# ZhenlongYuan/DVP-MVS

Hardware: AMD Instinct MI355X
Metric: Mpixels/sec/PatchMatch-iteration (higher is better)
Workload: dtype f32

## Files before the change

### __graft_entry__.py

```python
import importlib
import os
import subprocess
import sys

ROOT = os.path.dirname(os.path.abspath(__file__))
if ROOT not in sys.path:
    sys.path.insert(0, ROOT)


def build() -> None:
    subprocess.check_call(["make", "-s", "-C", os.path.join(ROOT, "dvp-mvs_amd", "csrc")])
    host = os.path.join(ROOT, "dvp-mvs_amd", "host")
    if os.path.exists(os.path.join(host, "Makefile")):
        subprocess.check_call(["make", "-s", "-C", host])
    subprocess.check_call(["make", "-s", "-C", os.path.join(ROOT, "oracle")])
    subprocess.check_call(["make", "-s", "-C", os.path.join(ROOT, "tests", "emul")])
    subprocess.check_call(["make", "-s", "-C", os.path.join(ROOT, "tests", "host")])
    subprocess.check_call(["make", "-s", "-C", os.path.join(ROOT, "tests", "half16")])
    subprocess.check_call(["make", "-s", "-C", os.path.join(ROOT, "tests", "jpeg_host")])
    subprocess.check_call(["make", "-s", "-C", os.path.join(ROOT, "tests", "edges_host")])
    subprocess.check_call(["make", "-s", "-C", os.path.join(ROOT, "tests", "viewclean_host")])
    subprocess.check_call(["make", "-s", "-C", os.path.join(ROOT, "tests", "labels_host")])
    subprocess.check_call(["make", "-s", "-C", os.path.join(ROOT, "tests", "pyramid_host")])
    subprocess.check_call(["make", "-s", "-C", os.path.join(ROOT, "tests", "prior_host")])
    subprocess.check_call(["make", "-s", "-C", os.path.join(ROOT, "tests", "reuse_host")])
    subprocess.check_call(["make", "-s", "-C", os.path.join(ROOT, "tests", "devmem_host")])
    subprocess.check_call(["make", "-s", "-C", os.path.join(ROOT, "tests", "jpeg_dec_host")])
    subprocess.check_call(["make", "-s", "-C", os.path.join(ROOT, "tests", "convert_host")])
    subprocess.check_call(["make", "-s", "-C", os.path.join(ROOT, "tests", "undistort_host")])
    pkg = importlib.import_module("dvp-mvs_amd")
    lib = pkg.get_capi().lib()
    missing = [s for s in pkg.get_capi().EXPORTS + pkg.get_capi().EXPORTS_WITH_DIGITS if not hasattr(lib, s)]
    if missing:
        raise RuntimeError("libdvp_mvs_hip.so lacks symbols: %s" % missing)


def smoke() -> None:
    import numpy as np
    pkg = importlib.import_module("dvp-mvs_amd")
    synth, capi = pkg.synth, pkg.get_capi()
    from oracle import oracle as O
    W, H, S = 96, 64, 3
    sc = synth.make_scene(W, H, S)
    p = synth.default_params(S + 1, max_iterations=1, state=synth.FIRST_INIT, use_APD=0)
    p["depth_min"] = np.float32(2.5) * np.float32(0.6)
    p["depth_max"] = np.float32(6.5) * np.float32(1.2)
    state = dict(planes=np.zeros((H * W, 4), np.float32), edge=sc["edge"], label=sc["label"],
                 radius=np.full(H * W, 5, np.int32))
    g = capi.from_scene(sc, p, device=0)
    g.upload_state(**state)
    g.run_patchmatch()
    o = O.from_scene(sc, p)
    o.upload_state(**state)
    o.run_patchmatch()
    pg, po = g.get("planes"), o.get("planes")
    same = (pg.view(np.uint32) == po.view(np.uint32)) | (np.isnan(pg) & np.isnan(po))
    if not same.all():
        raise AssertionError("smoke: HIP planes differ from the oracle in %d values" % int((~same).sum()))
    for n in ("selected_views", "weak_info", "radius"):
        if not (g.get(n) == o.get(n)).all():
            raise AssertionError("smoke: %s differs from the oracle" % n)
    print("smoke ok: %dx%d S=%d bit-exact vs oracle; total %.2f ms" % (W, H, S, g.timings()["total_ms"]))


if __name__ == "__main__":
    build()
    if os.path.exists("/dev/kfd"):
        smoke()
```

### dvp-mvs_amd/csrc/dvp_engine.hip

```cpp
#include "dvp_stages.hpp"
#include "dvp_jpeg_enc.h"
#include "dvp_edges_run.h"
#include "dvp_viewclean_run.h"
#include "dvp_prior_run.h"
#include "dvp_pyramid_run.h"
#include <hip/hip_runtime.h>
#include <cstdlib>
#include <string>
#include <vector>
#include <cstdio>
#include <cstring>
#include <mutex>
#include <condition_variable>
#include <thread>
#include <chrono>
#include <algorithm>
#include <cmath>

using namespace dvp;

struct LaunchArgs {
	int tiles_x, tiles, rows, half, colour, iter;
};

// ... 520 lines not shown
}

extern "C" __global__ void __launch_bounds__(256) dvp_gen_candidates_views(const Dev d, const LaunchArgs a) {
	int px, py;
	if (block_to_pixel(blockIdx.x, threadIdx.x & 63, threadIdx.x >> 6, a.tiles_x, a.tiles, a.rows, 0, 0, d.width, d.height, &px, &py))
		gen_candidates_views_px<kCandGroup>(d, px, py, (int)blockIdx.y * kCandGroup);
}
extern "C" __global__ void __launch_bounds__(256) dvp_gen_candidates_views_list(const Dev d, const unsigned* list, const unsigned* n_list) {
	const unsigned t = blockIdx.x * 256 + threadIdx.x;
	if (t >= *n_list) return;
	const int center = (int)list[t];
	const int py = center / d.width, px = center - py * d.width;
	gen_candidates_views_px<kCandGroup>(d, px, py, (int)blockIdx.y * kCandGroup);
}

extern "C" __global__ void __launch_bounds__(256) dvp_anchor_mask(const Dev d, const ListArgs a, uint8_t* mask) {
	const int t = blockIdx.x * 256 + threadIdx.x;
	if (t >= a.count) return;
	const int center = d.weak_list[a.base + t];
	const s2* nb = d.neighbours + (size_t)d.neighbours_map[center] * DVP_NEIGHBOUR_NUM;
	for (int k = 1; k < DVP_NEIGHBOUR_NUM; ++k) {
		const s2 q = nb[k];
		if (q.x >= 0 && q.y >= 0 && q.x < d.width && q.y < d.height) mask[(size_t)q.y * d.width + q.x] = 1;
	}
}
extern "C" __global__ void __launch_bounds__(256) dvp_mask_compact(const uint8_t* mask, size_t L, unsigned* list, unsigned* n_list) {
	const size_t p = (size_t)blockIdx.x * 256 + threadIdx.x;
	const bool go = p < L && mask[p] != 0;
	const unsigned long long m = __ballot(go);
	if (!m) return;
	const int lane = threadIdx.x & 63;
	unsigned base = 0;
	if (lane == __builtin_ctzll(m)) base = atomicAdd(n_list, (unsigned)__popcll(m));
	base = __shfl(base, __builtin_ctzll(m), 64);
	if (go) list[base + __popcll(m & ((1ull << lane) - 1ull))] = (unsigned)p;
}
extern "C" __global__ void __launch_bounds__(256) dvp_gen_candidates_list(const Dev d, const unsigned* list, const unsigned* n_list) {
	const unsigned t = blockIdx.x * 256 + threadIdx.x;
	if (t >= *n_list) return;
	const int center = (int)list[t];
	const int py = center / d.width, px = center - py * d.width;
	gen_candidates_px(d, px, py, (int)blockIdx.y);
}

extern "C" __global__ void dvp_pack_bits_transposed(const uint8_t* __restrict__ map, uint32_t* __restrict__ bits, int W, int H, int tiles_x, size_t words, int equals) {
	const size_t w = (size_t)blockIdx.x * blockDim.x + threadIdx.x;
	if (w < words) bits[w] = pack_edge_word_t(map, W, H, tiles_x, w, equals);
}

extern "C" __global__ void dvp_edge_cell_counts(const Dev d) {
	const int c = blockIdx.x * blockDim.x + threadIdx.x;
	if (c >= d.sat_cells_x * d.sat_cells_y) return;
	const int cy = c / d.sat_cells_x, cx = c - cy * d.sat_cells_x;
	int n = 0;
	for (int r = 0; r < 8; ++r) {
		const int y = cy * 8 + r;
		if (y >= d.height) break;
		const unsigned w = d.edge_bits[(size_t)(((y >> 5) * d.edge_tiles_x + (cx >> 2)) * 32 + (y & 31))];
		n += __popc((w >> ((cx & 3) * 8)) & 255u);
	}
	d.edge_sat[(cy + 1) * (d.sat_cells_x + 1) + cx + 1] = n;
}
extern "C" __global__ void dvp_edge_sat_rows(const Dev d) {
	const int r = blockIdx.x * blockDim.x + threadIdx.x;
	if (r > d.sat_cells_y) return;
	int* row = d.edge_sat + (size_t)r * (d.sat_cells_x + 1);
	int acc = 0;
	for (int x = 0; x <= d.sat_cells_x; ++x) { acc += (r == 0 || x == 0) ? 0 : row[x]; row[x] = acc; }
}
extern "C" __global__ void dvp_edge_sat_cols(const Dev d) {
	const int x = blockIdx.x * blockDim.x + threadIdx.x;
	if (x > d.sat_cells_x) return;
	const int P = d.sat_cells_x + 1;
	int acc = 0;
	for (int r = 0; r <= d.sat_cells_y; ++r) { acc += d.edge_sat[(size_t)r * P + x]; d.edge_sat[(size_t)r * P + x] = acc; }
}

extern "C" __global__ void __launch_bounds__(256) dvp_strong_search(const Dev d, const LaunchArgs a) {
	int px, py;
	if (block_to_pixel(blockIdx.x, threadIdx.x & 63, threadIdx.x >> 6, a.tiles_x, a.tiles, a.rows, a.half, a.colour, d.width, d.height, &px, &py))
		strong_search_px(d, px, py);
}

extern "C" __global__ void __launch_bounds__(256) dvp_strong_plan(const Dev d, const LaunchArgs a) {
	int px, py;
	if (block_to_pixel(blockIdx.x, threadIdx.x & 63, threadIdx.x >> 6, a.tiles_x, a.tiles, a.rows, a.half, a.colour, d.width, d.height, &px, &py) &&
	    d.weak_info[px + py * d.width] != DVP_WEAK)
		strong_plan_px(d, px, py);
}

extern "C" __global__ void __launch_bounds__(256) dvp_edge_rays(const Dev d, int what) {
	edge_ray_line(d, blockIdx.y, blockIdx.x * blockDim.x + threadIdx.x, what);
}

constexpr int kWeakTile = 16, kWeakSuper = 64, kWeakChunk = 1024;
DVP_HD void weak_slot_origin(int slot, int supers_x, int* tx, int* ty) {
	const int super = slot >> 4, t = slot & 15;
	*tx = (super % supers_x) * kWeakSuper + (t & 3) * kWeakTile;
	*ty = (super / supers_x) * kWeakSuper + (t >> 2) * kWeakTile;
}
extern "C" __global__ void __launch_bounds__(256) dvp_weak_counts(const uint8_t* __restrict__ weak, int W, int H, int supers_x, int n_slots, int n_chunks, int* __restrict__ counts) {
	const int lane = threadIdx.x & 63;
	const int unit = blockIdx.x * 4 + (threadIdx.x >> 6);
	if (unit < n_slots) {
		int tx, ty;
		weak_slot_origin(unit, supers_x, &tx, &ty);
		int nb = 0, nr = 0;
		for (int step = 0; step < 4; ++step) {
			const int x = tx + (lane & 15), y = ty + step * 4 + (lane >> 4);
			const bool wk = x < W && y < H && weak[(size_t)y * W + x] == DVP_WEAK;
			nb += __popcll(__ballot(wk && !((x + y) & 1)));
			nr += __popcll(__ballot(wk && ((x + y) & 1)));
		}
		if (lane == 0) { counts[unit] = nb; counts[n_slots + unit] = nr; }
	} else if (unit < n_slots + n_chunks) {
		const int chunk = unit - n_slots;
		const size_t L = (size_t)W * H;
		int n = 0;
		for (int step = 0; step < kWeakChunk / 64; ++step) {
			const size_t i = (size_t)chunk * kWeakChunk + step * 64 + lane;
			n += __popcll(__ballot(i < L && weak[i] == DVP_WEAK));
		}
		if (lane == 0) counts[2 * n_slots + chunk] = n;
	}
}
extern "C" __global__ void __launch_bounds__(1024) dvp_scan3(int* __restrict__ data, int s0, int s1, int s2, int s3, int* __restrict__ totals) {
	__shared__ int part[1024];
	__shared__ int carry;
	const int starts[4] = { s0, s1, s2, s3 };
	const int lo = starts[blockIdx.x], hi = starts[blockIdx.x + 1];
	if (threadIdx.x == 0) carry = 0;
	__syncthreads();
	for (int base = lo; base < hi; base += 1024) {
		const int i = base + (int)threadIdx.x;
		const int v = i < hi ? data[i] : 0;
		part[threadIdx.x] = v;
		__syncthreads();
		for (int off = 1; off < 1024; off <<= 1) {
			const int add = threadIdx.x >= (unsigned)off ? part[threadIdx.x - off] : 0;
			__syncthreads();
			part[threadIdx.x] += add;
			__syncthreads();
		}
		if (i < hi) data[i] = carry + part[threadIdx.x] - v;
		__syncthreads();
		if (threadIdx.x == 1023) carry += part[1023];
		__syncthreads();
	}
	if (threadIdx.x == 0) totals[blockIdx.x] = carry;
}
extern "C" __global__ void __launch_bounds__(256) dvp_weak_fill(const uint8_t* __restrict__ weak, int W, int H, int supers_x, int n_slots, int n_chunks,
                                                               const int* __restrict__ offs, const int* __restrict__ totals, int* __restrict__ list, int* __restrict__ map) {
	const int lane = threadIdx.x & 63;
	const int unit = blockIdx.x * 4 + (threadIdx.x >> 6);
	const unsigned long long below = (1ull << lane) - 1ull;
	if (unit < n_slots) {
		int tx, ty;
		weak_slot_origin(unit, supers_x, &tx, &ty);
		int ob = offs[unit], orr = totals[0] + offs[n_slots + unit];
		for (int step = 0; step < 4; ++step) {
			const int x = tx + (lane & 15), y = ty + step * 4 + (lane >> 4);
			const bool wk = x < W && y < H && weak[(size_t)y * W + x] == DVP_WEAK;
			const bool red = (x + y) & 1;
			const unsigned long long mb = __ballot(wk && !red), mr = __ballot(wk && red);
			if (wk) list[red ? orr + __popcll(mr & below) : ob + __popcll(mb & below)] = y * W + x;
			ob += __popcll(mb);
			orr += __popcll(mr);
// ... 908 lines not shown
		make_sector_taps(p->weak_radius, &taps, &start);
		if (dalloc(c, &c->sector_taps, taps.size(), false) || dalloc(c, &c->sector_start, start.size(), false)) return 1;
		HIP_TRY(c, hipMemcpyAsync(c->sector_taps, taps.data(), taps.size() * 4, hipMemcpyHostToDevice, c->stream));
		HIP_TRY(c, hipMemcpyAsync(c->sector_start, start.data(), start.size() * 4, hipMemcpyHostToDevice, c->stream));
		HIP_TRY(c, hipStreamSynchronize(c->stream));
		c->lut_radius = p->weak_radius;
	}
	sync_dev_struct(c);
	return 0;
}
int dvp_set_seed(dvp_ctx* c, uint64_t seed) { c->d.seed = seed; return 0; }
int dvp_set_sampler(dvp_ctx* c, int s) { c->d.sampler = s ? 1 : 0; bump_reuse_epoch(c); return 0; }
int dvp_set_profiling(dvp_ctx* c, int on) { c->profiling = on != 0; sync_dev_struct(c); return 0; }


static size_t alloc_group_or_fall_back(dvp_ctx* c, std::initializer_list<AllocReq> reqs, const char* hook, bool* fits, const char* msg, double gb, size_t retry_bytes = 0) {
	void* got[4] = { nullptr, nullptr, nullptr, nullptr };
	const AllocReq* r = reqs.begin();
	const size_t n = reqs.size();
	size_t first = r[0].bytes;
	bool ok = n <= 4 && !(hook && getenv(hook));
	for (size_t i = 0; i < n && ok; ++i) {
		if (!r[i].p) continue;
		ok = hipMalloc(&got[i], r[i].bytes) == hipSuccess;
		if (!ok && i == 0 && retry_bytes) { (void)hipGetLastError(); first = retry_bytes; ok = hipMalloc(&got[0], first) == hipSuccess; }
		if (!ok) got[i] = nullptr;
		else if (r[i].zero) ok = hipMemsetAsync(got[i], 0, r[i].bytes, c->stream) == hipSuccess;
	}
	if (!ok) {
		(void)hipGetLastError();
		for (void* q : got) if (q) (void)hipFree(q);
		*fits = false;
		if (msg) fprintf(stderr, msg, gb);
	}
	else for (size_t i = 0; i < n; ++i) if (r[i].p) { *r[i].p = got[i]; c->allocs.push_back(got[i]); }
	sync_dev_struct(c);
	return ok ? first : 0;
}

static int grow_anchor_table(dvp_ctx* c, size_t wc) {
	const size_t need = wc * (size_t)(c->NI - 1) * kAnchors;
	if (anchor_table_off(c) || need <= c->anchor_tab_alloc) return 0;
	HIP_TRY(c, hipStreamSynchronize(c->stream));
	dfree(c, &c->anchor_tab);
	c->anchor_tab_alloc = 0;
	c->anchor_tab_alloc = alloc_group_or_fall_back(c, { areq(&c->anchor_tab, (need + need / 2) * sizeof(AnchorRec)) }, nullptr, &c->anchor_tab_fits,
		"dvp: no room for the weak update's anchor table (%.1f GB); forming the reference side per item\n", (double)need * sizeof(AnchorRec) / 1e9,
		need * sizeof(AnchorRec)) / sizeof(AnchorRec);
	return 0;
}
static int ensure_anchor_table(dvp_ctx* c, int covered_rows) {
	if (anchor_table_off(c) || c->anchor_tab_valid) return 0;
	const int wc = c->d.weak_black + c->d.weak_red;
	if (grow_anchor_table(c, (size_t)wc)) return 1;
	if (anchor_table_off(c)) return 0;
	c->anchor_tab_valid = true;
	sync_dev_struct(c);
	ListArgs la;
	la.base = 0; la.count = wc; la.iter = 0; la.covered_rows = covered_rows;
	const long long n = (long long)wc * (c->NI - 1) * kAnchors;
	if (n > 0) {
		hipLaunchKernelGGL(dvp_weak_anchor_table, dim3((unsigned)((n + 255) / 256)), dim3(256), 0, c->stream, c->d, la);
		HIP_TRY(c, hipGetLastError());
	}
	return 0;
}

static int grow_weak_phase_buffers(dvp_ctx* c, size_t wc) {
	if (!c->sw.weak_phased || !c->weak_phase_fits || wc <= c->weak_phase_alloc) return 0;
	HIP_TRY(c, hipStreamSynchronize(c->stream));
	dfree(c, &c->weak_rec); dfree(c, &c->weak_ctab); dfree(c, &c->weak_ev);
	c->weak_phase_alloc = 0;
	const size_t cap = std::min<size_t>(c->L, wc + wc / 2), S = (size_t)c->NI - 1;
	if (alloc_group_or_fall_back(c, { areq(&c->weak_rec, cap * sizeof(WeakRec)), areq(&c->weak_ctab, cap * kTaps * kTaps * sizeof(f2)), areq(&c->weak_ev, cap * 8 * S * sizeof(float)) },
			"DVP_TEST_WEAK_PHASE_ALLOC_FAIL", &c->weak_phase_fits, "dvp: no room for the phased weak update's hand-over buffers (%.2f GB); using the one-wave kernel\n", (double)cap * (sizeof(WeakRec) + 288 + 32 * S) / 1e9))
		c->weak_phase_alloc = cap;
	return 0;
}

static void ensure_strong_reuse_buffers(dvp_ctx* c) {
	if (c->reuse_costs || !c->sw.strong_reuse || !c->reuse_fits || strong_form(c->sw, c->NI - 1, c->split_fits, false, 0).kernel != STRONG_SPLIT) return;
	const size_t L = c->L, vec = (size_t)kSlotCount * (c->NI - 1) * L * sizeof(float) + 64 ;
	const size_t Lh = (size_t)((c->W + 1) / 2) * c->H;
	alloc_group_or_fall_back(c, { areq(&c->reuse_costs, vec), areq(&c->reuse_keys, L * kSlotCount * sizeof(PlaneKey)), areq(&c->reuse_hdr, L * sizeof(ReuseHdr), true),
			c->strong_rec ? AllocReq{} : areq(&c->strong_rec, (size_t)SR_FIELDS * Lh * sizeof(*c->strong_rec)) },
		"DVP_TEST_REUSE_ALLOC_FAIL", &c->reuse_fits, "dvp: no room for the strong update's plane cache (%.1f GB); every visit evaluates all its planes\n", (double)(vec + L * (kSlotCount * sizeof(PlaneKey) + sizeof(ReuseHdr))) / 1e9);
}
static void ensure_strong_split_buffers(dvp_ctx* c) {
	if (c->slot_costs || strong_form(c->sw, c->NI - 1, c->split_fits, false, 0).kernel != STRONG_SPLIT) return;
	if (!getenv("DVP_TEST_SPLIT_ALLOC_FAIL")) {
		ensure_strong_reuse_buffers(c);
		if (c->reuse_costs) return;
	}
	const size_t Lh = (size_t)((c->W + 1) / 2) * c->H;
	alloc_group_or_fall_back(c, { areq(&c->slot_costs, (size_t)kSlotCount * (c->NI - 1) * Lh * sizeof(*c->slot_costs) + 64 ),
			areq(&c->strong_rec, (size_t)SR_FIELDS * Lh * sizeof(*c->strong_rec)) },
		"DVP_TEST_SPLIT_ALLOC_FAIL", &c->split_fits, "dvp: no room for the split strong update's cost buffer (%.1f GB); using the monolithic kernel\n", (double)kSlotCount * (c->NI - 1) * Lh * 4 / 1e9);
}
static void ensure_sweep_buffers(dvp_ctx* c) {
	if (c->sweep_cost || !c->sw.sweep_split || !c->sweep_fits) return;
	const size_t L = c->L;
	c->sweep_band_rows = sweep_band_rows(c->sw, c->W, c->H, c->NI - 1);
	const size_t band_px = c->sweep_band_rows > 0 ? (size_t)c->sweep_band_rows * c->W : L;
	alloc_group_or_fall_back(c, { areq(&c->sweep_rec, 2 * L * sizeof(f4)), areq(&c->sweep_pc, 61 * L * sizeof(float)), areq(&c->sweep_cost, sweep_cost_floats(band_px, c->NI - 1) * sizeof(float)) },
		"DVP_TEST_SWEEP_ALLOC_FAIL", &c->sweep_fits, "dvp: no room for the view-compacted DepthToWeak's cost buffer (%.1f GB); using the fused kernel\n", (double)(c->NI - 1) * kSweepFields * L * 4 / 1e9);
}


#define DVP_PICK(NAME, SUF) (c->d.sampler ? NAME##_exact##SUF : NAME##SUF)
#define DVP_PICK_FMT(NAME, TAIL) (fmt == 1 ? DVP_PICK(NAME, _u8##TAIL) : (fmt == 2 ? DVP_PICK(NAME, _f16##TAIL) : DVP_PICK(NAME, TAIL)))

static LaunchArgs make_args(const LaunchGeom& g, int colour, int iter) {
	LaunchArgs a;
	a.tiles_x = g.tiles_x; a.tiles = g.tiles; a.rows = g.rows; a.half = g.half ? 1 : 0;
	a.colour = colour; a.iter = iter;
	return a;
}

static void launch_gen_candidates(dvp_ctx* c, hipStream_t stream, const Dev& d, unsigned blocks, const LaunchArgs& a, const unsigned* list = nullptr, const unsigned* n_list = nullptr) {
	const bool all = gen_candidates_all_views(d);
	const dim3 grid(blocks, all ? (unsigned)((c->NI - 1 + kCandGroup - 1) / kCandGroup) : (unsigned)(c->NI - 1)), block(256);
	if (list) hipLaunchKernelGGL(all ? dvp_gen_candidates_views_list : dvp_gen_candidates_list, grid, block, 0, stream, d, list, n_list);
	else hipLaunchKernelGGL(all ? dvp_gen_candidates_views : dvp_gen_candidates, grid, block, 0, stream, d, a);
}

static int launch_strong_prep(dvp_ctx* c, const LaunchGeom& g, const LaunchArgs& a) {
	EventPair prep;
	prep.stage = DVP_ST_STRONG_PREP;
	HIP_TRY(c, hipEventCreate(&prep.a));
	HIP_TRY(c, hipEventCreate(&prep.b));
	HIP_TRY(c, hipEventRecord(prep.a, c->stream));
	HIP_TRY(c, hipMemcpyAsync(c->planes_snap, c->planes, c->L * 16, hipMemcpyDeviceToDevice, c->stream));
	HIP_TRY(c, hipMemcpyAsync(c->costs_snap, c->costs, c->L * 4, hipMemcpyDeviceToDevice, c->stream));
	ensure_strong_split_buffers(c);
	hipLaunchKernelGGL(dvp_strong_search, dim3(g.grid()), dim3(256), 0, c->stream, c->d, a);
	if (strong_form(c->sw, c->NI - 1, c->split_fits, c->d.reuse_hdr != nullptr, 0).plan) hipLaunchKernelGGL(dvp_strong_plan, dim3(g.grid()), dim3(256), 0, c->stream, c->d, a);
	HIP_TRY(c, hipGetLastError());
	HIP_TRY(c, hipEventRecord(prep.b, c->stream));
	c->events.push_back(prep);
	return 0;
}

static int launch_strong_update(dvp_ctx* c, const LaunchGeom& g, const LaunchArgs& a) {
	const dim3 grid(g.grid()), block(256);
	const dim3 wave_grid((unsigned)((g.grid() + 7) / 8 * 32)), wave_block(64);
	ensure_strong_split_buffers(c);
	const StrongForm f = strong_form(c->sw, c->NI - 1, c->split_fits, c->d.reuse_hdr != nullptr, (unsigned long long)c->pitch * (c->H + 2 * kImgPad) * 8 * c->NI);
	switch (f.kernel) {
	case STRONG_SPLIT:
		if (f.eval_items) hipLaunchKernelGGL(DVP_PICK(dvp_strong_eval_items, ), wave_grid, wave_block, 0, c->stream, c->d, a);
		else hipLaunchKernelGGL(DVP_PICK(dvp_strong_eval, ), wave_grid, wave_block, 0, c->stream, c->d, a);
		hipLaunchKernelGGL(f.decide == 4 ? dvp_strong_decide_v4 : f.decide == 6 ? dvp_strong_decide_v6 : f.decide == 8 ? dvp_strong_decide_v8 : f.decide == 10 ? dvp_strong_decide_v10 :
		                   f.decide == 12 ? dvp_strong_decide_v12 : f.decide == 16 ? dvp_strong_decide_v16 : dvp_strong_decide_wide, grid, block, 0, c->stream, c->d, a);
		if (f.refine_lanes) hipLaunchKernelGGL(DVP_PICK(dvp_strong_refine_lanes, ), wave_grid, wave_block, 0, c->stream, c->d, a);
		else hipLaunchKernelGGL(DVP_PICK(dvp_strong_refine, ), wave_grid, wave_block, 0, c->stream, c->d, a);
		break;
	case STRONG_MONO_V8: hipLaunchKernelGGL(DVP_PICK(dvp_strong_update_v8, ), grid, block, 0, c->stream, c->d, a); break;
	case STRONG_MONO_V16: hipLaunchKernelGGL(DVP_PICK(dvp_strong_update_v16, ), grid, block, 0, c->stream, c->d, a); break;
	case STRONG_MONO: hipLaunchKernelGGL(DVP_PICK(dvp_strong_update, ), grid, block, 0, c->stream, c->d, a); break;
	}
	HIP_TRY(c, hipGetLastError());
	return 0;
}

static int launch_weak_update(dvp_ctx* c, ListArgs la) {
	if (ensure_anchor_table(c, la.covered_rows)) return 1;
	if (c->d.anchor_tab && grow_weak_phase_buffers(c, (size_t)(c->d.weak_black + c->d.weak_red))) return 1;
// ... 687 lines not shown
```

### dvp-mvs_amd/csrc/dvp_strong.hpp

```cpp
#ifndef DVP_STRONG_HPP_
#define DVP_STRONG_HPP_

#include "dvp_ncc.hpp"

namespace dvp {

DVP_HD void sort_small(float* v, int n) {
	for (int i = 1; i < n; i++) {
		const float tmp = v[i];
		int j = i;
		for (; j >= 1 && tmp < v[j - 1]; j--) v[j] = v[j - 1];
		v[j] = tmp;
	}
}

DVP_HD f4 random_normal_yzl_sel(const Dev& d, int px, int py, Rng& rng, float depth, uint32_t sel) {
	const int W = d.width, H = d.height;
	const DvpCamera rc = load_camera(d, 0);
	f3 vd[20];
	{
		const f4 v0 = view_direction(rc, px, py, depth);
		vd[0] = mk3(v0.x, v0.y, v0.z);
	}
	int index = 1;
// ... 438 lines not shown
			}
			Rng rd(d.seed, (uint32_t)center, rng_site(PH_STRONG, iter, SUB_DEPTH_RAND));
			Rng rn(d.seed, (uint32_t)center, rng_site(PH_STRONG, iter, SUB_NORMAL));
			Rng rp(d.seed, (uint32_t)center, rng_site(PH_STRONG, iter, SUB_DEPTH_PERT));
			const float depth_rand = rd.uniform() * (P.depth_max - P.depth_min) + P.depth_min;
			if (selected_views_written) d.selected_views[center] = sel_mask;
			const f4 n_rand = random_normal_yzl(d, px, py, rn, depth_now);
			const float dmin_p = (1 - 0.02f) * depth_now, dmax_p = (1 + 0.02f) * depth_now;
			const float depth_pert = rp.uniform() * (dmax_p - dmin_p) + dmin_p;
			f4 n_pert = plane_now;
			normalize3(&n_pert);
			ref_depths[0] = depth_rand; ref_normals[0] = plane_now;
			ref_depths[1] = depth_now;  ref_normals[1] = n_rand;
			ref_depths[2] = depth_rand; ref_normals[2] = n_rand;
			ref_depths[3] = depth_now;  ref_normals[3] = n_pert;
			ref_depths[4] = depth_now;  ref_normals[4] = n_pert;
			ref_depths[5] = depth_pert; ref_normals[5] = plane_now;
		} else {
			float tc = 0.0f;
			for (int j = 0; j < S; ++j)
				if (vw[j] > 0) tc += vw[j] * cv[j];
			tc /= weight_norm;
			const float db = depth_from_plane(rc, plane, px, py);
			if (db >= P.depth_min && db <= P.depth_max && tc < cost_now) {
				depth_now = db;
				plane_now = plane;
				cost_now = tc;
			}
		}
	}

	if (P.state == DVP_REFINE_INIT) {
		if (cost_now < costs_center - 0.1) {
			costs_center = cost_now;
			d.planes[center] = plane_now;
		}
	} else {
		costs_center = cost_now;
		d.planes[center] = plane_now;
	}
	d.costs[center] = costs_center;
}

constexpr int kSlotCur = 16;
constexpr int kSlotCount = 17;
enum { SR_PLANE = 0, SR_DEPTH = 4, SR_COST = 5, SR_CENTER = 6, SR_DRAND = 7, SR_DPERT = 8, SR_NRAND = 9, SR_DUP = 12 , SR_FIELDS = 15 };
DVP_HD size_t half_index(const Dev& d, int px, int py) { return (size_t)py * d.half_w + (size_t)(px >> 1); }
#ifndef DVP_SLOT_LAYOUT
#define DVP_SLOT_LAYOUT 1
#endif
DVP_HD int slot_place(int slot) {
#if DVP_SLOT_LAYOUT
	return slot < 8 ? 2 * slot : (slot < 16 ? 2 * (slot - 8) + 1 : slot);
#else
	return slot;
#endif
}
DVP_HD size_t slot_cost_index(const Dev& d, int slot, int v, int px, int py) {
	const size_t Lh = (size_t)d.half_w * (size_t)d.height;
	const int S = d.params.num_images - 1;
#if DVP_SLOT_LAYOUT
	return (half_index(d, px, py) * kSlotCount + (size_t)slot_place(slot)) * (size_t)S + (size_t)v;
#else
	return (size_t)(slot * S + v) * Lh + half_index(d, px, py);
#endif
}
struct SlotCostView { const float* base; size_t slot_stride, view_stride; };
DVP_HD SlotCostView slot_cost_view(const Dev& d, int px, int py) {
	const size_t Lh = (size_t)d.half_w * (size_t)d.height;
	const int S = d.params.num_images - 1;
	SlotCostView r;
#if DVP_SLOT_LAYOUT
	r.base = d.slot_costs + half_index(d, px, py) * kSlotCount * (size_t)S;
	r.slot_stride = (size_t)S;
	r.view_stride = 1;
#else
	r.base = d.slot_costs + half_index(d, px, py);
	r.slot_stride = (size_t)S * Lh;
	r.view_stride = Lh;
#endif
	return r;
}
DVP_HD bool same_plane_bits(const f4 a, const f4 b) {
	return f32_bits(a.x) == f32_bits(b.x) && f32_bits(a.y) == f32_bits(b.y) && f32_bits(a.z) == f32_bits(b.z) && f32_bits(a.w) == f32_bits(b.w);
}
DVP_HD uint32_t strong_slot_planes(const Dev& d, int center, f4 pl[kSlotCount]) {
	const size_t L = (size_t)d.width * d.height;
	uint32_t have = 0;
#pragma unroll
	for (int slot = 0; slot < kSlotCount; ++slot) {
		const int pos = slot < 16 ? d.search_pos[(size_t)slot * L + center] : center;
		pl[slot] = mk4(0.0f, 0.0f, 0.0f, 0.0f);
		if (pos >= 0) { pl[slot] = d.planes_snap[pos]; have |= 1u << slot; }
	}
	return have;
}
DVP_HD uint32_t strong_slot_sources_of(const f4 pl[kSlotCount], uint32_t have, uint32_t w[3]) {
	uint32_t uniq = 0;
	w[0] = w[1] = w[2] = 0;
#pragma unroll
	for (int slot = 0; slot < kSlotCount; ++slot) {
		int src = slot;
#pragma unroll
		for (int u = slot - 1; u >= 0; --u)
			if (((have >> u) & 1u) && same_plane_bits(pl[u], pl[slot])) src = u;
		if (!((have >> slot) & 1u)) continue;
		if (src == slot) uniq |= 1u << slot;
		if (slot < 8) w[0] |= (uint32_t)src << (4 * slot);
		else if (slot < 16) w[1] |= (uint32_t)src << (4 * (slot - 8));
		else w[2] = (uint32_t)src;
	}
	return uniq;
}
DVP_HD uint32_t strong_slot_sources(const Dev& d, int center, uint32_t w[3]) {
	f4 pl[kSlotCount];
	const uint32_t have = strong_slot_planes(d, center, pl);
	return strong_slot_sources_of(pl, have, w);
}
DVP_HD int strong_slot_source(uint32_t w0, uint32_t w1, uint32_t w2, int slot) {
	return slot < 8 ? (int)((w0 >> (4 * slot)) & 15u) : slot < 16 ? (int)((w1 >> (4 * (slot - 8))) & 15u) : (int)w2;
}
constexpr uint32_t kPlaceMask = (1u << kSlotCount) - 1u;
DVP_HD int strong_slot_place_of(uint32_t w0, uint32_t w1, uint32_t w2, int slot) {
	return slot < 6 ? (int)((w0 >> (5 * slot)) & 31u) : slot < 12 ? (int)((w1 >> (5 * (slot - 6))) & 31u) : (int)((w2 >> (5 * (slot - 12))) & 31u);
}
DVP_HD void strong_source_places(const uint32_t src[3], uint32_t place_w[3]) {
	place_w[0] = place_w[1] = place_w[2] = 0;
#pragma unroll
	for (int s = 0; s < kSlotCount; ++s)
		place_w[s / 6] |= (uint32_t)slot_place(strong_slot_source(src[0], src[1], src[2], s)) << (5 * (s % 6));
}
DVP_HD PlaneKey plane_key(const f4 p) {
	PlaneKey k;
	k.w[0] = f32_bits(p.x); k.w[1] = f32_bits(p.y); k.w[2] = f32_bits(p.z); k.w[3] = f32_bits(p.w);
	return k;
}
DVP_HD uint32_t strong_reuse_plan(const f4 pl[kSlotCount], uint32_t uniq, const uint32_t src[3], PlaneKey* keys, ReuseHdr* hdr,
                                  uint32_t epoch, int radius, uint32_t place_w[3]) {
	const ReuseHdr h = *hdr;
	const uint32_t valid = (h.epoch == epoch && h.radius == (uint32_t)radius) ? (h.valid & kPlaceMask) : 0u;
	int place[kSlotCount];
#pragma unroll
	for (int s = 0; s < kSlotCount; ++s) place[s] = -1;
	uint32_t held = 0;
	if (valid) {
#pragma unroll
		for (int p = 0; p < kSlotCount; ++p) {
			if (!((valid >> p) & 1u)) continue;
			const PlaneKey k = keys[p];
#pragma unroll
			for (int s = 0; s < kSlotCount; ++s) {
				if (!((uniq >> s) & 1u) || place[s] >= 0) continue;
				if (k.w[0] == f32_bits(pl[s].x) && k.w[1] == f32_bits(pl[s].y) && k.w[2] == f32_bits(pl[s].z) && k.w[3] == f32_bits(pl[s].w)) { place[s] = p; held |= 1u << p; }
			}
		}
	}
	uint32_t free_places = kPlaceMask & ~held, eval = 0;
#pragma unroll
	for (int s = 0; s < kSlotCount; ++s) {
		if (!((uniq >> s) & 1u) || place[s] >= 0) continue;
		const int p = dvp_ctz(free_places);
		free_places &= free_places - 1;
		place[s] = p;
		eval |= 1u << s;
		keys[p] = plane_key(pl[s]);
	}
	place_w[0] = place_w[1] = place_w[2] = 0;
#pragma unroll
	for (int s = 0; s < kSlotCount; ++s) {
		const int from = strong_slot_source(src[0], src[1], src[2], s);
		int p = 0;
#pragma unroll
		for (int u = 0; u <= s; ++u)
			if (u == from && place[u] >= 0) p = place[u];
		place_w[s / 6] |= (uint32_t)p << (5 * (s % 6));
	}
	ReuseHdr o;
	o.valid = kPlaceMask & ~free_places; o.radius = (uint32_t)radius; o.epoch = epoch; o.eval = eval;
	*hdr = o;
	return eval;
}
DVP_HD void strong_plan_px(const Dev& d, int px, int py) {
	const int center = py * d.width + px;
	f4 pl[kSlotCount];
	const uint32_t have = strong_slot_planes(d, center, pl);
	uint32_t src[3], pw[3];
	const uint32_t uniq = strong_slot_sources_of(pl, have, src);
	strong_reuse_plan(pl, uniq, src, d.reuse_keys + (size_t)center * kSlotCount, d.reuse_hdr + center, d.reuse_epoch, d.radius[center], pw);
	const size_t Lh = (size_t)d.half_w * (size_t)d.height;
	uint32_t* dup = reinterpret_cast<uint32_t*>(d.strong_rec) + half_index(d, px, py);
	dup[SR_DUP * Lh] = pw[0]; dup[(SR_DUP + 1) * Lh] = pw[1]; dup[(SR_DUP + 2) * Lh] = pw[2];
}
template <int SMP>
DVP_HD void strong_eval_item(const Dev& d, const PatchCtx& c, int px, int py, int slot, bool store, unsigned long long* nevals) {
	const int W = d.width;
	const int center = py * W + px;
	const int S = d.params.num_images - 1;
	const size_t L = (size_t)W * d.height;
	const int pos = slot < 16 ? d.search_pos[(size_t)slot * L + center] : center;
	const f4 plane = d.planes_snap[pos];
	const bool reuse = d.reuse_costs != nullptr;
	float* const buf = reuse ? d.reuse_costs : d.slot_costs;
	int at = slot_place(slot);
	if (reuse) {
		const size_t Lh = (size_t)d.half_w * (size_t)d.height;
		const int word = (slot >= 6) + (slot >= 12);
		const uint32_t pw = reinterpret_cast<const uint32_t*>(d.strong_rec)[(size_t)(SR_DUP + word) * Lh + half_index(d, px, py)];
		at = (int)((pw >> (5 * (slot - 6 * word))) & 31u);
	}
	for (int v = 0; v < S; ++v) {
		const float cost = ncc_old<SMP>(d, c, px, py, v + 1, plane);
#if DVP_SLOT_LAYOUT
		const size_t rec = reuse ? (size_t)center : half_index(d, px, py);
		if (store) DVP_NT_STORE(4, &buf[(rec * kSlotCount + (size_t)at) * (size_t)S + (size_t)v], cost);
#else
		if (store) DVP_NT_STORE(4, &buf[reuse ? ((size_t)center * kSlotCount + (size_t)at) * (size_t)S + (size_t)v : slot_cost_index(d, slot, v, px, py)], cost);
#endif
	}
	if (nevals && store) *nevals += (unsigned long long)S;
}
template <int SMP>
DVP_HD void strong_eval_px(const Dev& d, int px, int py, PatchTab tab, unsigned long long* nevals) {
	const int W = d.width;
	const int center = py * W + px;
	PatchCtx c;
	{
		int radius, inc;
		patch_geometry(d, center, &radius, &inc);
		build_patch_ctx(d, px, py, radius, inc, 0, tab, &c);
	}
	uint32_t uniq;
	if (d.reuse_hdr) uniq = d.reuse_hdr[center].eval;
	else {
		uint32_t src[3], w[3];
		uniq = strong_slot_sources(d, center, src);
		strong_source_places(src, w);
		const size_t Lh = (size_t)d.half_w * (size_t)d.height, hi = half_index(d, px, py);
		uint32_t* dup = reinterpret_cast<uint32_t*>(d.strong_rec) + hi;
		dup[SR_DUP * Lh] = w[0]; dup[(SR_DUP + 1) * Lh] = w[1]; dup[(SR_DUP + 2) * Lh] = w[2];
	}
	for (uint32_t m = uniq; m; m &= m - 1) strong_eval_item<SMP>(d, c, px, py, dvp_ctz(m), true, nevals);
}

template <int MV>
DVP_HD void load_slot_costs(const float* sc, size_t view_stride, int S, float* out) {
#if defined(__HIP_DEVICE_COMPILE__) && DVP_SLOT_LAYOUT
	typedef float f4v __attribute__((ext_vector_type(4), aligned(4)));
	constexpr int Q = (MV + 3) / 4;
	f4v q[Q];
#pragma unroll
	for (int i = 0; i < Q; ++i) q[i] = DVP_NT_LOAD(8, &reinterpret_cast<const f4v*>(sc)[i]);
#pragma unroll
	for (int v = 0; v < MV; ++v) out[v] = v < S ? q[v >> 2][v & 3] : 0.0f;
#else
#pragma unroll
	for (int v = 0; v < MV; ++v) out[v] = v < S ? sc[(size_t)v * view_stride] : 0.0f;
#endif
}

DVP_HD void strong_decide_wide_px(const Dev& d, int px, int py, int iter);
template <int MV>
DVP_HD void strong_decide_px(const Dev& d, int px, int py, int iter) {
#if !defined(__HIP_DEVICE_COMPILE__)
	if (d.params.num_images - 1 > MV) { strong_decide_wide_px(d, px, py, iter); return; }
#endif
	const int W = d.width;
	const int center = py * W + px;
	const DvpParams& P = d.params;
	const DvpCamera rc = load_camera(d, 0);
	const int S = P.num_images - 1;
	const bool reuse = d.reuse_costs != nullptr;
	SlotCostView cv;
// ... 1128 lines not shown
```

Before: 60.91.

## Match strong-plan reuse slots by fingerprint with coalesced key layout

The strong plan kernel now hashes each cached plane key and each candidate plane into a 30-bit fingerprint and matches slots by comparing fingerprints. It falls back to the full bitwise key scan only when a fingerprint match fails verification. The reuse keys move from a per-pixel array of records to a slot-major, colour-split layout, so neighbouring threads read adjacent keys. The change also makes the plane gather branchless, loads the search positions up front, and sets a minimum-occupancy launch bound on the plan kernel. The cost is extra hashing arithmetic and possible register pressure, aimed at cutting the divergent nested compare loops and the strided key loads.

```diff
diff --git a/__graft_entry__.py b/__graft_entry__.py
--- a/__graft_entry__.py
+++ b/__graft_entry__.py
@@ -24,6 +24,7 @@
     subprocess.check_call(["make", "-s", "-C", os.path.join(ROOT, "tests", "pyramid_host")])
     subprocess.check_call(["make", "-s", "-C", os.path.join(ROOT, "tests", "prior_host")])
     subprocess.check_call(["make", "-s", "-C", os.path.join(ROOT, "tests", "reuse_host")])
+    subprocess.check_call(["make", "-s", "-C", os.path.join(ROOT, "tests", "plan_fp_host")])
     subprocess.check_call(["make", "-s", "-C", os.path.join(ROOT, "tests", "devmem_host")])
     subprocess.check_call(["make", "-s", "-C", os.path.join(ROOT, "tests", "jpeg_dec_host")])
     subprocess.check_call(["make", "-s", "-C", os.path.join(ROOT, "tests", "convert_host")])
diff --git a/dvp-mvs_amd/csrc/dvp_engine.hip b/dvp-mvs_amd/csrc/dvp_engine.hip
--- a/dvp-mvs_amd/csrc/dvp_engine.hip
+++ b/dvp-mvs_amd/csrc/dvp_engine.hip
@@ -626,7 +626,10 @@
 		strong_search_px(d, px, py);
 }
 
-extern "C" __global__ void __launch_bounds__(256) dvp_strong_plan(const Dev d, const LaunchArgs a) {
+#ifndef DVP_LB_PLAN
+#define DVP_LB_PLAN 3
+#endif
+extern "C" __global__ void __launch_bounds__(256, DVP_LB_PLAN) dvp_strong_plan(const Dev d, const LaunchArgs a) {
 	int px, py;
 	if (block_to_pixel(blockIdx.x, threadIdx.x & 63, threadIdx.x >> 6, a.tiles_x, a.tiles, a.rows, a.half, a.colour, d.width, d.height, &px, &py) &&
 	    d.weak_info[px + py * d.width] != DVP_WEAK)
@@ -1701,7 +1704,7 @@
 	if (c->reuse_costs || !c->sw.strong_reuse || !c->reuse_fits || strong_form(c->sw, c->NI - 1, c->split_fits, false, 0).kernel != STRONG_SPLIT) return;
 	const size_t L = c->L, vec = (size_t)kSlotCount * (c->NI - 1) * L * sizeof(float) + 64 ;
 	const size_t Lh = (size_t)((c->W + 1) / 2) * c->H;
-	alloc_group_or_fall_back(c, { areq(&c->reuse_costs, vec), areq(&c->reuse_keys, L * kSlotCount * sizeof(PlaneKey)), areq(&c->reuse_hdr, L * sizeof(ReuseHdr), true),
+	alloc_group_or_fall_back(c, { areq(&c->reuse_costs, vec), areq(&c->reuse_keys, 2 * Lh * kSlotCount * sizeof(PlaneKey) ), areq(&c->reuse_hdr, L * sizeof(ReuseHdr), true),
 			c->strong_rec ? AllocReq{} : areq(&c->strong_rec, (size_t)SR_FIELDS * Lh * sizeof(*c->strong_rec)) },
 		"DVP_TEST_REUSE_ALLOC_FAIL", &c->reuse_fits, "dvp: no room for the strong update's plane cache (%.1f GB); every visit evaluates all its planes\n", (double)(vec + L * (kSlotCount * sizeof(PlaneKey) + sizeof(ReuseHdr))) / 1e9);
 }
diff --git a/dvp-mvs_amd/csrc/dvp_strong.hpp b/dvp-mvs_amd/csrc/dvp_strong.hpp
--- a/dvp-mvs_amd/csrc/dvp_strong.hpp
+++ b/dvp-mvs_amd/csrc/dvp_strong.hpp
@@ -544,16 +544,21 @@
 	return r;
 }
 DVP_HD bool same_plane_bits(const f4 a, const f4 b) {
-	return f32_bits(a.x) == f32_bits(b.x) && f32_bits(a.y) == f32_bits(b.y) && f32_bits(a.z) == f32_bits(b.z) && f32_bits(a.w) == f32_bits(b.w);
+	return ((f32_bits(a.x) ^ f32_bits(b.x)) | (f32_bits(a.y) ^ f32_bits(b.y)) | (f32_bits(a.z) ^ f32_bits(b.z)) | (f32_bits(a.w) ^ f32_bits(b.w))) == 0;
 }
 DVP_HD uint32_t strong_slot_planes(const Dev& d, int center, f4 pl[kSlotCount]) {
 	const size_t L = (size_t)d.width * d.height;
+	int pos[kSlotCount];
+#pragma unroll
+	for (int slot = 0; slot < kSlotCount; ++slot) pos[slot] = slot < 16 ? d.search_pos[(size_t)slot * L + center] : center;
 	uint32_t have = 0;
 #pragma unroll
 	for (int slot = 0; slot < kSlotCount; ++slot) {
-		const int pos = slot < 16 ? d.search_pos[(size_t)slot * L + center] : center;
-		pl[slot] = mk4(0.0f, 0.0f, 0.0f, 0.0f);
-		if (pos >= 0) { pl[slot] = d.planes_snap[pos]; have |= 1u << slot; }
+		const uint32_t keep = ~(uint32_t)(pos[slot] >> 31);
+		const f4 p = d.planes_snap[((uint32_t)pos[slot] & keep) | ((uint32_t)center & ~keep)];
+		pl[slot] = mk4(__builtin_bit_cast(float, f32_bits(p.x) & keep), __builtin_bit_cast(float, f32_bits(p.y) & keep),
+		               __builtin_bit_cast(float, f32_bits(p.z) & keep), __builtin_bit_cast(float, f32_bits(p.w) & keep));
+		if (pos[slot] >= 0) have |= 1u << slot;
 	}
 	return have;
 }
@@ -565,7 +570,7 @@
 		int src = slot;
 #pragma unroll
 		for (int u = slot - 1; u >= 0; --u)
-			if (((have >> u) & 1u) && same_plane_bits(pl[u], pl[slot])) src = u;
+			if ((int)((have >> u) & 1u) & (int)same_plane_bits(pl[u], pl[slot])) src = u;
 		if (!((have >> slot) & 1u)) continue;
 		if (src == slot) uniq |= 1u << slot;
 		if (slot < 8) w[0] |= (uint32_t)src << (4 * slot);
@@ -597,59 +602,104 @@
 	k.w[0] = f32_bits(p.x); k.w[1] = f32_bits(p.y); k.w[2] = f32_bits(p.z); k.w[3] = f32_bits(p.w);
 	return k;
 }
-DVP_HD uint32_t strong_reuse_plan(const f4 pl[kSlotCount], uint32_t uniq, const uint32_t src[3], PlaneKey* keys, ReuseHdr* hdr,
-                                  uint32_t epoch, int radius, uint32_t place_w[3]) {
+#ifndef DVP_PLAN_FP_MASK
+#define DVP_PLAN_FP_MASK 0x3FFFFFFFu
+#endif
+DVP_HD uint32_t plan_rotl(uint32_t x, int r) { return (x << r) | (x >> (32 - r)); }
+DVP_HD uint32_t plane_fingerprint(uint32_t w0, uint32_t w1, uint32_t w2, uint32_t w3) {
+	const uint32_t h = (w0 ^ plan_rotl(w1, 13)) + (plan_rotl(w2, 26) ^ plan_rotl(w3, 7));
+	return (h ^ (h >> 15)) & 0x3FFFFFFFu & DVP_PLAN_FP_MASK;
+}
+struct ReuseOld { uint32_t valid, fp[kSlotCount]; };
+DVP_HD ReuseOld strong_reuse_old(const PlaneKey* keys, size_t key_stride, const ReuseHdr* hdr, uint32_t epoch, int radius) {
 	const ReuseHdr h = *hdr;
-	const uint32_t valid = (h.epoch == epoch && h.radius == (uint32_t)radius) ? (h.valid & kPlaceMask) : 0u;
+	ReuseOld o;
+	o.valid = (h.epoch == epoch && h.radius == (uint32_t)radius) ? (h.valid & kPlaceMask) : 0u;
+#pragma unroll
+	for (int p = 0; p < kSlotCount; ++p) {
+		const PlaneKey k = keys[(size_t)p * key_stride];
+		o.fp[p] = plane_fingerprint(k.w[0], k.w[1], k.w[2], k.w[3]) | ((~o.valid >> p & 1u) << 31);
+	}
+	return o;
+}
+DVP_HD bool key_is_plane(const PlaneKey k, const f4 p) {
+	return k.w[0] == f32_bits(p.x) && k.w[1] == f32_bits(p.y) && k.w[2] == f32_bits(p.z) && k.w[3] == f32_bits(p.w);
+}
+DVP_HD uint32_t strong_reuse_plan_old(const f4 pl[kSlotCount], uint32_t uniq, const uint32_t src[3], PlaneKey* keys, size_t key_stride, ReuseHdr* hdr,
+                                      const ReuseOld& old, uint32_t epoch, int radius, uint32_t place_w[3]) {
 	int place[kSlotCount];
 #pragma unroll
-	for (int s = 0; s < kSlotCount; ++s) place[s] = -1;
+	for (int s = 0; s < kSlotCount; ++s) {
+		const uint32_t fp = plane_fingerprint(f32_bits(pl[s].x), f32_bits(pl[s].y), f32_bits(pl[s].z), f32_bits(pl[s].w)) | ((~uniq >> s & 1u) << 30);
+		int cand = -1;
+#pragma unroll
+		for (int p = kSlotCount - 1; p >= 0; --p)
+			if (old.fp[p] == fp) cand = p;
+		place[s] = cand;
+	}
+	bool collision = false;
+#pragma unroll
+	for (int s = 0; s < kSlotCount; ++s)
+		if (place[s] >= 0 && !key_is_plane(keys[(size_t)place[s] * key_stride], pl[s])) collision = true;
+	if (collision) {
+#pragma unroll
+		for (int s = 0; s < kSlotCount; ++s) place[s] = -1;
+#pragma unroll 1
+		for (int p = 0; p < kSlotCount; ++p) {
+			if (!((old.valid >> p) & 1u)) continue;
+			const PlaneKey k = keys[(size_t)p * key_stride];
+#pragma unroll
+			for (int s = 0; s < kSlotCount; ++s)
+				if (((uniq >> s) & 1u) && place[s] < 0 && key_is_plane(k, pl[s])) place[s] = p;
+		}
+	}
 	uint32_t held = 0;
-	if (valid) {
-#pragma unroll
-		for (int p = 0; p < kSlotCount; ++p) {
-			if (!((valid >> p) & 1u)) continue;
-			const PlaneKey k = keys[p];
-#pragma unroll
-			for (int s = 0; s < kSlotCount; ++s) {
-				if (!((uniq >> s) & 1u) || place[s] >= 0) continue;
-				if (k.w[0] == f32_bits(pl[s].x) && k.w[1] == f32_bits(pl[s].y) && k.w[2] == f32_bits(pl[s].z) && k.w[3] == f32_bits(pl[s].w)) { place[s] = p; held |= 1u << p; }
-			}
-		}
-	}
+#pragma unroll
+	for (int s = 0; s < kSlotCount; ++s) held |= 1u << (place[s] & 31);
 	uint32_t free_places = kPlaceMask & ~held, eval = 0;
+	unsigned long long lo = 0;
+	uint32_t hi = 0;
 #pragma unroll
 	for (int s = 0; s < kSlotCount; ++s) {
-		if (!((uniq >> s) & 1u) || place[s] >= 0) continue;
-		const int p = dvp_ctz(free_places);
-		free_places &= free_places - 1;
-		place[s] = p;
-		eval |= 1u << s;
-		keys[p] = plane_key(pl[s]);
+		if (!((uniq >> s) & 1u)) continue;
+		int p = place[s];
+		if (p < 0) {
+			p = dvp_ctz(free_places);
+			free_places &= free_places - 1;
+			eval |= 1u << s;
+			keys[(size_t)p * key_stride] = plane_key(pl[s]);
+		}
+		if (s < 12) lo |= (unsigned long long)p << (5 * s);
+		else hi |= (uint32_t)p << (5 * (s - 12));
 	}
 	place_w[0] = place_w[1] = place_w[2] = 0;
 #pragma unroll
 	for (int s = 0; s < kSlotCount; ++s) {
 		const int from = strong_slot_source(src[0], src[1], src[2], s);
-		int p = 0;
-#pragma unroll
-		for (int u = 0; u <= s; ++u)
-			if (u == from && place[u] >= 0) p = place[u];
-		place_w[s / 6] |= (uint32_t)p << (5 * (s % 6));
+		const uint32_t p = (from < 12 ? (uint32_t)(lo >> (5 * from)) : hi >> (5 * ((from - 12) & 7))) & 31u;
+		place_w[s / 6] |= p << (5 * (s % 6));
 	}
 	ReuseHdr o;
 	o.valid = kPlaceMask & ~free_places; o.radius = (uint32_t)radius; o.epoch = epoch; o.eval = eval;
 	*hdr = o;
 	return eval;
 }
+DVP_HD uint32_t strong_reuse_plan(const f4 pl[kSlotCount], uint32_t uniq, const uint32_t src[3], PlaneKey* keys, ReuseHdr* hdr,
+                                  uint32_t epoch, int radius, uint32_t place_w[3]) {
+	const ReuseOld old = strong_reuse_old(keys, 1, hdr, epoch, radius);
+	return strong_reuse_plan_old(pl, uniq, src, keys, 1, hdr, old, epoch, radius, place_w);
+}
 DVP_HD void strong_plan_px(const Dev& d, int px, int py) {
 	const int center = py * d.width + px;
+	const size_t Lh = (size_t)d.half_w * (size_t)d.height, key_stride = 2 * Lh;
+	PlaneKey* const keys = d.reuse_keys + (size_t)((px + py) & 1) * Lh + half_index(d, px, py);
+	const int radius = d.radius[center];
+	const ReuseOld old = strong_reuse_old(keys, key_stride, d.reuse_hdr + center, d.reuse_epoch, radius);
 	f4 pl[kSlotCount];
 	const uint32_t have = strong_slot_planes(d, center, pl);
 	uint32_t src[3], pw[3];
 	const uint32_t uniq = strong_slot_sources_of(pl, have, src);
-	strong_reuse_plan(pl, uniq, src, d.reuse_keys + (size_t)center * kSlotCount, d.reuse_hdr + center, d.reuse_epoch, d.radius[center], pw);
-	const size_t Lh = (size_t)d.half_w * (size_t)d.height;
+	strong_reuse_plan_old(pl, uniq, src, keys, key_stride, d.reuse_hdr + center, old, d.reuse_epoch, radius, pw);
 	uint32_t* dup = reinterpret_cast<uint32_t*>(d.strong_rec) + half_index(d, px, py);
 	dup[SR_DUP * Lh] = pw[0]; dup[(SR_DUP + 1) * Lh] = pw[1]; dup[(SR_DUP + 2) * Lh] = pw[2];
 }
```

New measurement: 61.30 (median of 6 runs). About the same (+0.6%).
